# fperezgamonal/flownet2-tf

Hardware: AMD Instinct MI355X
Metric: forward pairs/sec at 512x384 (FlowNet2) (higher is better)
Workload: dtype f16x2 (split fp16 hi+lo operands, 3 fp16 MFMAs per product, fp32 accumulate); 1 GPU; FlowNet2 forward, batch=4 synthetic 512x384 pairs per GPU, seeded synthetic weights; pairs_per_gpu=4, parallelism=dp1 (no collective)

## Files before the change

flownet2-tf_amd/csrc/conv.hip:

```cpp
#include "conv_common.h"
#include <cstdlib>

namespace fn2 {

template <typename T, typename OutT, int TC, int WC, int WP>
__global__ void __launch_bounds__(256) conv_igemm_kernel(const ConvArgs p) {
  constexpr int CH = 16 / (int)sizeof(T);
  constexpr int BC = WC * TC * 16;
  constexpr int BP = WP * 64;
  constexpr int NT = 256;
  static_assert(WC * WP == 4, "4 waves per block");
  constexpr int NPR = BP / 64;
  constexpr int NWR = (BC * 4 + NT - 1) / NT;
  constexpr int WSWZ_BIT = (TC == 4) ? 5 : (TC == 2) ? 4 : 3;
  __shared__ uint4 lds[2][(BC + BP) * 4];

  const int tid = threadIdx.x, lane = tid & 63, wave = tid >> 6;
  const int wc = wave / WP, wp = wave % WP;
  const int cid = tid & 3;

  int pad_y = p.pad, pad_x = p.pad, oy_off = 0, ox_off = 0, osc = 1;
  const T* wgt = reinterpret_cast<const T*>(p.wgt);
  const int phase = blockIdx.z / p.splitk, split = blockIdx.z - phase * p.splitk;
  if (p.deconv) {
// ... 160 lines not shown
  for (int pt = 0; pt < 4; ++pt) {
    const int m = m0 + wp * 64 + pt * 16 + fi;
    if (m >= p.M) continue;
    const int n = m / (p.OH * p.OW);
    const int rem = m - n * (p.OH * p.OW);
    const int oy = rem / p.OW, ox = rem - oy * p.OW;
    OutT* po = out + (((size_t)n * p.out_H + (oy * osc + oy_off)) * p.out_W + (ox * osc + ox_off)) * p.out_cs +
               p.out_c0;
#pragma unroll
    for (int t = 0; t < TC; ++t) {
      float v[4];
      const int co = cout_base + t * 4;
#pragma unroll
      for (int r = 0; r < 4; ++r) {
        float x = acc[t][pt][r] * p.out_scale + bias[t][r];
        if constexpr (sizeof(OutT) == 4) {
          if (p.accum && co + r < p.Cout) x += load_elem<OutT>(po + co + r);
          if (co + r < p.Cout) x = act_grad<OutT>(p, out, po + co + r, co + r, x);
        }
        if (p.act == FN2_ACT_LEAKY) x = leaky(x);
        v[r] = x;
      }
      if (p.vec_ok && co + 3 < p.Cout) {
        store4<OutT>(po + co, v[0], v[1], v[2], v[3]);
      } else {
#pragma unroll
        for (int r = 0; r < 4; ++r)
          if (co + r < p.Cout) store_elem<OutT>(po + co + r, v[r]);
      }
    }
  }
}

template <typename OutT>
__global__ void __launch_bounds__(256) splitk_finalize_kernel(const float* __restrict__ ws, const float* __restrict__ bias,
                                                              OutT* __restrict__ out, long npix, int ws_cs, int splitk,
                                                              int Cout, int out_cs, int out_c0, int act, int vec_ok,
                                                              float out_scale, int accum, const OutT* __restrict__ mask_y,
                                                              int mask_c0, int mask_c1, const float* __restrict__ up_src,
                                                              const float* __restrict__ up_w, const float* __restrict__ up_bias,
                                                              int up_c0, int out_H, int out_W) {
  const int groups = ws_cs / 4;
  const int groups_all = groups + (up_src != nullptr ? 1 : 0);
  const long total = npix * groups_all;
  const size_t slab = (size_t)npix * ws_cs;
  for (long i = (long)blockIdx.x * blockDim.x + threadIdx.x; i < total; i += (long)gridDim.x * blockDim.x) {
    const long pix = i / groups_all;
    const int co = (int)(i - pix * groups_all) * 4;
    if (co == groups * 4) {
      const int ox = (int)(pix % out_W), oy = (int)((pix / out_W) % out_H), n = (int)(pix / out_W / out_H);
      const int H = out_H >> 1, W = out_W >> 1;
      const int a = oy & 1, b = ox & 1, y = oy >> 1, x = ox >> 1;
      float r0 = up_bias ? up_bias[0] : 0.f, r1 = up_bias ? up_bias[1] : 0.f;
#pragma unroll
      for (int ty = 0; ty < 2; ++ty) {
        const int iy = y - 1 + a + ty, ky = 3 - a - 2 * ty;
        if (iy < 0 || iy >= H) continue;
#pragma unroll
        for (int tx = 0; tx < 2; ++tx) {
          const int ix = x - 1 + b + tx, kx = 3 - b - 2 * tx;
          if (ix < 0 || ix >= W) continue;
          const float2 v = *reinterpret_cast<const float2*>(up_src + (((long)n * H + iy) * W + ix) * 2);
          const float* ww = up_w + (ky * 4 + kx) * 4;
          r0 += v.x * ww[0] + v.y * ww[1];
          r1 += v.x * ww[2] + v.y * ww[3];
        }
      }
      OutT* pu = out + (size_t)pix * out_cs + up_c0;
      store_elem<OutT>(pu, r0);
      store_elem<OutT>(pu + 1, r1);
      continue;
    }
    float4 v = *reinterpret_cast<const float4*>(ws + pix * ws_cs + co);
    int s = 1;
    for (; s + 3 < splitk; s += 4) {
      float4 t[4];
#pragma unroll
      for (int u = 0; u < 4; ++u) t[u] = *reinterpret_cast<const float4*>(ws + (s + u) * slab + pix * ws_cs + co);
#pragma unroll
      for (int u = 0; u < 4; ++u) { v.x += t[u].x; v.y += t[u].y; v.z += t[u].z; v.w += t[u].w; }
    }
    for (; s < splitk; ++s) {
      const float4 t = *reinterpret_cast<const float4*>(ws + s * slab + pix * ws_cs + co);
      v.x += t.x; v.y += t.y; v.z += t.z; v.w += t.w;
    }
    float r[4] = {v.x, v.y, v.z, v.w};
    OutT* po = out + (size_t)pix * out_cs + out_c0 + co;
    const bool full = vec_ok && co + 3 < Cout;
    float old[4] = {0.f, 0.f, 0.f, 0.f}, yv[4] = {1.f, 1.f, 1.f, 1.f};
    const bool mask = mask_y != nullptr && co < mask_c1 && co + 4 > mask_c0;
    if constexpr (sizeof(OutT) == 4) {
      if (full) {
        if (accum) load4<OutT>(po, old);
        if (mask) load4<OutT>(mask_y + (size_t)pix * out_cs + out_c0 + co, yv);
      } else {
#pragma unroll
        for (int j = 0; j < 4; ++j)
          if (co + j < Cout) {
            if (accum) old[j] = load_elem<OutT>(po + j);
            if (mask) yv[j] = load_elem<OutT>(mask_y + (size_t)pix * out_cs + out_c0 + co + j);
          }
      }
    }
#pragma unroll
    for (int j = 0; j < 4; ++j) {
      r[j] *= out_scale;
      if (bias != nullptr && co + j < Cout) r[j] += bias[co + j];
      if constexpr (sizeof(OutT) == 4) {
        if (accum) r[j] += old[j];
        if (mask && co + j >= mask_c0 && co + j < mask_c1) r[j] *= yv[j] > 0.f ? 1.f : (yv[j] < 0.f ? 0.1f : 0.55f);
      }
      if (act == FN2_ACT_LEAKY) r[j] = leaky(r[j]);
    }
    if (vec_ok && co + 3 < Cout) {
      store4<OutT>(po, r[0], r[1], r[2], r[3]);
    } else {
#pragma unroll
// ... 179 lines not shown
    for (int idx = tid; idx < HY * HX * 9; idx += 256) {
      const int p = idx / 9, j = idx - p * 9;
      const int hy = p / HX, hx = p - hy * HX;
      const int gy = y0 + hy, gx = x0 + hx;
      float2 v = make_float2(0.f, 0.f);
      if (gy >= 0 && gy < H && gx >= 0 && gx < W)
        v = *reinterpret_cast<const float2*>(t + (((long)n * H + gy) * W + gx) * t_cs + 2 * j);
      sm[idx] = v;
    }
    __syncthreads();
    const int px = tid & (GT_X - 1);
#pragma unroll
    for (int r = 0; r < GT_Y / 4; ++r) {
      const int py = (tid >> 6) + 4 * r;
      const int oy = ty * GT_Y + py, ox = tx * GT_X + px;
      if (oy < H && ox < W) {
        float a0 = b0, a1 = b1;
#pragma unroll
        for (int ky = 0; ky < 3; ++ky)
#pragma unroll
          for (int kx = 0; kx < 3; ++kx) {
            const float2 v = sm[((py + ky) * HX + px + kx) * 9 + ky * 3 + kx];
            a0 += v.x; a1 += v.y;
          }
        *reinterpret_cast<float2*>(out + (((long)n * H + oy) * W + ox) * 2) = make_float2(a0, a1);
      }
    }
    __syncthreads();
  }
}

struct TailSrc { const float* t; int t_cs; int nslab; long slab; float scale; };

template <int NT, int TY, int TX, bool UP, typename OutT>
__global__ void __launch_bounds__(256) head_tail_kernel(const TailSrc ts, const float* __restrict__ bias,
                                                        float* __restrict__ pf, int N, int H, int W, int ring,
                                                        const float* __restrict__ up_w, const float* __restrict__ up_bias,
                                                        OutT* __restrict__ up, int up_cs, int up_c0) {
  constexpr int R = NT / 2, E = UP ? 1 : 0, HALO = R + E;
  constexpr int RW = TX + 2 * HALO, RH = TY + 2 * HALO, NTAP = NT * NT;
  constexpr int EW = TX + 2 * E, EH = TY + 2 * E;
  __shared__ float2 sm[RH * RW * NTAP];
  __shared__ float2 spf[EH * EW];
  __shared__ float sw[64];
  const int tid = threadIdx.x;
  if (UP && tid < 64) sw[tid] = up_w[tid];
  const int tiles_x = (W + TX - 1) / TX, tiles_y = (H + TY - 1) / TY;
  const float b0 = bias ? bias[0] : 0.f, b1 = bias ? bias[1] : 0.f;
  for (int blk = blockIdx.x; blk < N * tiles_y * tiles_x; blk += gridDim.x) {
    const int tx = blk % tiles_x, ty = (blk / tiles_x) % tiles_y, n = blk / (tiles_x * tiles_y);
    const int x0 = tx * TX - HALO, y0 = ty * TY - HALO;
    for (int idx = tid; idx < RH * RW * NTAP; idx += 256) {
      const int p = idx / NTAP, j = idx - p * NTAP;
      const int hy = p / RW, hx = p - hy * RW;
      const int gy = y0 + hy, gx = x0 + hx;
      float2 v = make_float2(0.f, 0.f);
      if (gy >= 0 && gy < H && gx >= 0 && gx < W) {
        const float* src = ts.t + (((long)n * H + gy) * W + gx) * ts.t_cs + 2 * j;
        v = *reinterpret_cast<const float2*>(src);
        for (int sl = 1; sl < ts.nslab; ++sl) {
          const float2 u = *reinterpret_cast<const float2*>(src + sl * ts.slab);
          v.x += u.x; v.y += u.y;
        }
        v.x *= ts.scale; v.y *= ts.scale;
      }
      sm[idx] = v;
    }
    __syncthreads();
    for (int e = tid; e < EH * EW; e += 256) {
      const int ey = e / EW, ex = e - ey * EW;
      const int oy = ty * TY - E + ey, ox = tx * TX - E + ex;
      float a0 = 0.f, a1 = 0.f;
      if (oy >= 0 && oy < H && ox >= 0 && ox < W) {
        const bool inner = ey >= E && ey < E + TY && ex >= E && ex < E + TX;
        float2* po = reinterpret_cast<float2*>(pf + (((long)n * H + oy) * W + ox) * 2);
        if (ring && (oy == 0 || oy == H - 1 || ox == 0 || ox == W - 1)) {
          const float2 v = *po;
          a0 = v.x; a1 = v.y;
        } else {
          a0 = b0; a1 = b1;
#pragma unroll
          for (int ky = 0; ky < NT; ++ky)
#pragma unroll
            for (int kx = 0; kx < NT; ++kx) {
// ... 19 lines not shown
          const int iy = y - 1 + a + tty, ky = 3 - a - 2 * tty;
          const int gy = ty * TY + iy;
          if (gy < 0 || gy >= H) continue;
#pragma unroll
          for (int ttx = 0; ttx < 2; ++ttx) {
            const int ix = x - 1 + b + ttx, kx = 3 - b - 2 * ttx;
            const int gx = tx * TX + ix;
            if (gx < 0 || gx >= W) continue;
            const float2 v = spf[(iy + E) * EW + ix + E];
            const float* ww = sw + (ky * 4 + kx) * 4;
            r0 += v.x * ww[0] + v.y * ww[1];
            r1 += v.x * ww[2] + v.y * ww[3];
          }
        }
        OutT* po = up + (((size_t)n * 2 * H + oy) * 2 * W + ox) * up_cs + up_c0;
        if constexpr (is_x2<OutT>::value) {
          const size_t addr = reinterpret_cast<size_t>(po);
          _Float16* g = reinterpret_cast<_Float16*>(addr & ~size_t(31));
          const int j = (int)((addr & 31) >> 2);
          typedef __attribute__((ext_vector_type(2))) _Float16 h2;
          const _Float16 h0 = (_Float16)r0, h1 = (_Float16)r1;
          *reinterpret_cast<h2*>(g + j) = h2{h0, h1};
          *reinterpret_cast<h2*>(g + 8 + j) = h2{(_Float16)(r0 - (float)h0), (_Float16)(r1 - (float)h1)};
        } else {
          store_elem<OutT>(po, r0);
          store_elem<OutT>(po + 1, r1);
        }
      }
    }
    __syncthreads();
  }
}

__global__ void __launch_bounds__(256) head_ring_kernel(const x2_t* __restrict__ in, int in_cs, int in_c0, int cin_groups,
                                                        const float* __restrict__ wc, const float* __restrict__ bc,
                                                        float* __restrict__ pf, int N, int H, int W) {
  const int lane = threadIdx.x & 63;
  const long wave = ((long)blockIdx.x * blockDim.x + threadIdx.x) >> 6;
  const long nwaves = ((long)gridDim.x * blockDim.x) >> 6;
  const int ring = 2 * W + 2 * (H - 2);
  const int nitems = 25 * cin_groups;
  const size_t case_stride = (size_t)nitems * 8 * 2;
  for (long m = wave; m < (long)N * ring; m += nwaves) {
    const int n = (int)(m / ring), r = (int)(m - (long)n * ring);
    int y, x;
    if (r < W) { y = 0; x = r; }
    else if (r < 2 * W) { y = H - 1; x = r - W; }
    else { const int q = r - 2 * W; y = 1 + (q >> 1); x = (q & 1) ? W - 1 : 0; }
    const int cy = y == 0 ? 0 : (y == H - 1 ? 2 : 1), cx = x == 0 ? 0 : (x == W - 1 ? 2 : 1);
    const int cs = 3 * cy + cx;
    const float* w = wc + (size_t)cs * case_stride;
    float a0 = 0.f, a1 = 0.f;
    for (int q = lane; q < nitems; q += 64) {
      const int tap = q / cin_groups, gi = q - tap * cin_groups;
      const int ky = tap / 5, kx = tap - ky * 5;
      const int iy = y + ky - 2, ix = x + kx - 2;
      if (iy < 0 || iy >= H || ix < 0 || ix >= W) continue;
      const uint4* src = reinterpret_cast<const uint4*>(in + (((size_t)n * H + iy) * W + ix) * in_cs + in_c0 + gi * 8);
      float xv[8];
      join8(src[0], src[1], xv);
      const float* u = w + (size_t)q * 16;
#pragma unroll
      for (int j = 0; j < 8; ++j) {
        a0 += xv[j] * u[2 * j];
        a1 += xv[j] * u[2 * j + 1];
      }
    }
#pragma unroll
    for (int off = 32; off > 0; off >>= 1) {
      a0 += __shfl_xor(a0, off, 64);
      a1 += __shfl_xor(a1, off, 64);
    }
    if (lane == 0)
      *reinterpret_cast<float2*>(pf + (((size_t)n * H + y) * W + x) * 2) = make_float2(a0 + bc[2 * cs], a1 + bc[2 * cs + 1]);
  }
}

template <typename OutT>
__global__ void __launch_bounds__(256) upsample_flow_kernel(const float* __restrict__ in,
                                                            const float* __restrict__ w, const float* __restrict__ bias,
                                                            OutT* __restrict__ out,
                                                            int N, int H, int W, int out_cs, int out_c0) {
  __shared__ float sw[64];
  if (threadIdx.x < 64) sw[threadIdx.x] = w[threadIdx.x];
  __syncthreads();
// ... 81 lines not shown
  if (g > 256L * 16) g = 256L * 16;
  if (g < 1) g = 1;
  return (int)g;
}

static int check_view(const fn2_tensor* t, const char* what) {
  FN2_REQUIRE(t && t->data, "%s: null tensor", what);
  FN2_REQUIRE(t->dtype >= FN2_F32 && t->dtype <= FN2_F16X2, "%s: bad dtype", what);
  FN2_REQUIRE(t->n >= 1 && t->h >= 1 && t->w >= 1 && t->c >= 1, "%s: bad dims", what);
  FN2_REQUIRE(t->c0 >= 0 && t->c0 + t->c <= t->cs, "%s: channel slice outside the buffer", what);
  return FN2_OK;
}

template <int NIMG>
static int pack_imgs(const float* i0, const float* i1, const fn2_tensor* out, int n, int n0, int pad, void* stream) {
  FN2_REQUIRE(pad >= 0 && out->h > 2 * pad && out->w > 2 * pad, "pack: bad border");
  FN2_REQUIRE(out->c0 % 8 == 0 && out->cs % 8 == 0 && out->c0 + 8 <= out->cs, "pack: needs an 8-channel aligned slot");
  const int h = out->h - 2 * pad, w = out->w - 2 * pad;
  const long npix = (long)n * h * w;
  const dim3 g(grid_for(npix, 256)), b(256);
  hipStream_t s = (hipStream_t)stream;
  if (out->dtype == FN2_F32)
    hipLaunchKernelGGL((pack_image_kernel<float, NIMG>), g, b, 0, s, i0, i1, (float*)out->data, n, h, w, n0, pad, out->cs, out->c0);
  else if (out->dtype == FN2_F16X2)
    hipLaunchKernelGGL((pack_image_kernel<x2_t, NIMG>), g, b, 0, s, i0, i1, (x2_t*)out->data, n, h, w, n0, pad, out->cs, out->c0);
  else if (out->dtype == FN2_BF16)
    hipLaunchKernelGGL((pack_image_kernel<bf16_t, NIMG>), g, b, 0, s, i0, i1, (bf16_t*)out->data, n, h, w, n0, pad, out->cs, out->c0);
  else
    hipLaunchKernelGGL((pack_image_kernel<f16_t, NIMG>), g, b, 0, s, i0, i1, (f16_t*)out->data, n, h, w, n0, pad, out->cs, out->c0);
  FN2_CHECK_LAUNCH("pack_image");
  return FN2_OK;
}

template <int NT, int TY, int TX, typename OutT>
void launch_head_tail(bool up, const TailSrc ts, const float* bias, float* pf, int n, int h, int w, int ring,
                      const float* up_w, const float* up_bias, void* up_data, int up_cs, int up_c0, hipStream_t s) {
  const long tiles = (long)n * ((h + TY - 1) / TY) * ((w + TX - 1) / TX);
  const dim3 grid((unsigned)std::min<long>(tiles, 1 << 16)), block(256);
  if (up)
    hipLaunchKernelGGL((head_tail_kernel<NT, TY, TX, true, OutT>), grid, block, 0, s, ts, bias, pf, n, h, w, ring, up_w,
                       up_bias, (OutT*)up_data, up_cs, up_c0);
  else
    hipLaunchKernelGGL((head_tail_kernel<NT, TY, TX, false, float>), grid, block, 0, s, ts, bias, pf, n, h, w, ring,
                       (const float*)nullptr, (const float*)nullptr, (float*)nullptr, 0, 0);
}
template <typename OutT>
void launch_head_tail_t(int taps, bool up, const TailSrc ts, const float* bias, float* pf, int n, int h, int w,
                        int ring, const float* up_w, const float* up_bias, void* up_data, int up_cs, int up_c0,
                        hipStream_t s) {
  const long big = (long)n * ((h + 7) / 8) * ((w + 63) / 64);
  if (taps == 3) {
    if (big >= 256) launch_head_tail<3, 8, 64, OutT>(up, ts, bias, pf, n, h, w, ring, up_w, up_bias, up_data, up_cs, up_c0, s);
    else launch_head_tail<3, 4, 32, OutT>(up, ts, bias, pf, n, h, w, ring, up_w, up_bias, up_data, up_cs, up_c0, s);
  } else {
    if (big >= 256) launch_head_tail<5, 8, 32, OutT>(up, ts, bias, pf, n, h, w, ring, up_w, up_bias, up_data, up_cs, up_c0, s);
    else launch_head_tail<5, 4, 32, OutT>(up, ts, bias, pf, n, h, w, ring, up_w, up_bias, up_data, up_cs, up_c0, s);
  }
}

}

using namespace fn2;

extern "C" {

int fn2_conv2d_plan(int in_dtype, int cin_pad, int cout, fn2_conv_plan* plan) {
  FN2_REQUIRE(plan, "conv2d_plan: null plan");
  FN2_REQUIRE(in_dtype >= FN2_F32 && in_dtype <= FN2_F16X2, "conv2d_plan: bad dtype");
  FN2_REQUIRE(cin_pad > 0 && cin_pad % 8 == 0 && cout >= 1, "conv2d_plan: cin_pad must be a positive multiple of 8");
  const int esz = dtype_size(in_dtype);
  if (cout == 2) {
    plan->layout = 0; plan->cout_tile = 16; plan->kstep_elems = 64 / esz;
    plan->wgt_dtype = in_dtype == FN2_F16X2 ? FN2_F32 : in_dtype;
    return FN2_OK;
  }
  if (conv_fast_ok(in_dtype, cin_pad, cout)) {
    plan->layout = 1; plan->cout_tile = cout > 64 ? 128 : cout > 32 ? 64 : 32; plan->kstep_elems = 128 / esz;
    plan->wgt_dtype = in_dtype;
    return FN2_OK;
  }
  if (in_dtype == FN2_F16X2)
    return fail(FN2_ERR_UNSUPPORTED, "split-fp16 inputs need cin_pad %% 32 == 0 (LDS-DMA kernel); got %d", cin_pad);
  plan->layout = 0; plan->cout_tile = cout > 64 ? 128 : cout > 32 ? 64 : cout > 16 ? 32 : 16;
  plan->kstep_elems = 64 / esz; plan->wgt_dtype = in_dtype;
  return FN2_OK;
}

}

// ... 340 lines not shown
      a.fh_w1 = ha.ksteps * 4 * 4;
      a.fh_groups = ha.cin_chunks >> 1;
      a.fh_bias = ha.bias;
      a.fh_out = reinterpret_cast<float*>(ha.out);
      a.fh_out_cs = ha.out_cs; a.fh_out_c0 = ha.out_c0;
      a.fh_scale = ha.out_scale;
    } else {
      rc = fn2_conv2d(h, stream);
      if (rc) return rc;
    }
  }
  if (d->wgt_layout >= 1) {
    a.ksteps = a.ksteps / 2;
    a.kper = cdiv(a.kper, 2);
    a.splitk = cdiv(a.ksteps, a.kper);
    if (a.splitk == 1) a.ws = nullptr;
    rc = launch_conv_fast(a, d->in.dtype, d->out.dtype, tile, phases, s);
  } else if (d->in.dtype == FN2_F32 && d->out.dtype == FN2_F16X2) rc = launch_conv<float, x2_t>(a, tile, phases, s);
  else if (d->in.dtype == FN2_F32) rc = launch_conv<float, float>(a, tile, phases, s);
  else if (d->in.dtype == FN2_BF16 && d->out.dtype == FN2_BF16) rc = launch_conv<bf16_t, bf16_t>(a, tile, phases, s);
  else if (d->in.dtype == FN2_BF16) rc = launch_conv<bf16_t, float>(a, tile, phases, s);
  else if (d->out.dtype == FN2_F16) rc = launch_conv<f16_t, f16_t>(a, tile, phases, s);
  else rc = launch_conv<f16_t, float>(a, tile, phases, s);
  if (rc || conv_name_sink().buf) return rc;
  if (a.splitk == 1) {
    if (d->up_src == nullptr || a.up_src != nullptr) return rc;
    fn2_tensor uv = d->out;
    uv.c = 2; uv.c0 = d->up_c0;
    return fn2_upsample_flow(d->up_src, d->up_w, d->up_bias, &uv, d->out.n, d->out.h / 2, d->out.w / 2, stream);
  }
  if ((a.dbg & 524288) || d->raw_partials) return rc;
  const long npix = (long)a.N * a.out_H * a.out_W;
  const int fgrid = grid_for(npix * (a.ws_cs / 4 + (d->up_src != nullptr ? 1 : 0)), 256);
  if (d->out.dtype == FN2_F32)
    hipLaunchKernelGGL(splitk_finalize_kernel<float>, dim3(fgrid), dim3(256), 0, s, a.ws, a.bias, (float*)a.out, npix,
                       a.ws_cs, a.splitk, a.Cout, a.out_cs, a.out_c0, a.act, a.vec_ok, a.out_scale, a.accum, (const float*)a.mask_y, a.mask_c0, a.mask_c1, d->up_src, d->up_w, d->up_bias, d->up_c0, a.out_H, a.out_W);
  else if (d->out.dtype == FN2_F16X2)
    hipLaunchKernelGGL(splitk_finalize_kernel<x2_t>, dim3(fgrid), dim3(256), 0, s, a.ws, a.bias, (x2_t*)a.out,
                       npix, a.ws_cs, a.splitk, a.Cout, a.out_cs, a.out_c0, a.act, a.vec_ok, a.out_scale, a.accum, (const x2_t*)a.mask_y, a.mask_c0, a.mask_c1, d->up_src, d->up_w, d->up_bias, d->up_c0, a.out_H, a.out_W);
  else if (d->out.dtype == FN2_BF16)
    hipLaunchKernelGGL(splitk_finalize_kernel<bf16_t>, dim3(fgrid), dim3(256), 0, s, a.ws, a.bias, (bf16_t*)a.out,
                       npix, a.ws_cs, a.splitk, a.Cout, a.out_cs, a.out_c0, a.act, a.vec_ok, a.out_scale, a.accum, (const bf16_t*)a.mask_y, a.mask_c0, a.mask_c1, d->up_src, d->up_w, d->up_bias, d->up_c0, a.out_H, a.out_W);
  else
    hipLaunchKernelGGL(splitk_finalize_kernel<f16_t>, dim3(fgrid), dim3(256), 0, s, a.ws, a.bias, (f16_t*)a.out,
                       npix, a.ws_cs, a.splitk, a.Cout, a.out_cs, a.out_c0, a.act, a.vec_ok, a.out_scale, a.accum, (const f16_t*)a.mask_y, a.mask_c0, a.mask_c1, d->up_src, d->up_w, d->up_bias, d->up_c0, a.out_H, a.out_W);
  FN2_CHECK_LAUNCH("splitk_finalize");
  return FN2_OK;
}

int fn2_flow_head_gather(const float* t, int t_cs, const float* bias, float* out, int n, int h, int w, void* stream) {
  FN2_REQUIRE(t && out, "flow_head_gather: null pointer");
  FN2_REQUIRE(t_cs >= 18 && t_cs % 2 == 0 && n >= 1 && h >= 1 && w >= 1, "flow_head_gather: t must hold 18 partials per pixel");
  const long tiles = (long)n * ((h + GT_Y - 1) / GT_Y) * ((w + GT_X - 1) / GT_X);
  if (tiles >= 1024)
    hipLaunchKernelGGL(flow_head_gather_kernel, dim3((unsigned)std::min<long>(tiles, 1 << 16)), dim3(256), 0,
                       (hipStream_t)stream, t, t_cs, bias, out, n, h, w);
  else
    hipLaunchKernelGGL(flow_head_gather_small_kernel, dim3(grid_for((long)n * h * w, 256)), dim3(256), 0,
                       (hipStream_t)stream, t, t_cs, bias, out, n, h, w);
  FN2_CHECK_LAUNCH("flow_head_gather");
  return FN2_OK;
}

int fn2_flow_head_tail(const float* t, int t_cs, int taps, const float* bias, float* pf, int n, int h, int w, int ring,
                       const float* up_w, const float* up_bias, const fn2_tensor* up_out, void* stream) {
  return fn2_flow_head_tail_slabs(t, t_cs, 1, 0, 1.f, taps, bias, pf, n, h, w, ring, up_w, up_bias, up_out, stream);
}

int fn2_flow_head_tail_slabs(const float* t, int t_cs, int nslab, int64_t slab_stride, float scale, int taps, const float* bias,
                             float* pf, int n, int h, int w, int ring, const float* up_w, const float* up_bias,
                             const fn2_tensor* up_out, void* stream) {
  FN2_REQUIRE(t && pf, "flow_head_tail: null pointer");
  FN2_REQUIRE(nslab >= 1 && (nslab == 1 || slab_stride >= (int64_t)n * h * w * t_cs), "flow_head_tail: bad slab geometry");
  const TailSrc ts{t, t_cs, nslab, (long)slab_stride, scale};
  FN2_REQUIRE(taps == 3 || taps == 5, "flow_head_tail: taps must be 3 or 5");
  FN2_REQUIRE(t_cs >= 2 * taps * taps && t_cs % 2 == 0 && n >= 1 && h >= 1 && w >= 1,
              "flow_head_tail: t must hold 2 * taps^2 partials per pixel");
  FN2_REQUIRE(!ring || (h >= 3 && w >= 3), "flow_head_tail: a border ring needs h, w >= 3");
  const bool up = up_w != nullptr;
  hipStream_t s = (hipStream_t)stream;
  if (!up) {
    launch_head_tail_t<float>(taps, false, ts, bias, pf, n, h, w, ring, nullptr, nullptr, nullptr, 0, 0, s);
  } else {
    int rc = check_view(up_out, "flow_head_tail upsample output");
    if (rc) return rc;
    FN2_REQUIRE(up_out->c == 2 && up_out->n == n && up_out->h == 2 * h && up_out->w == 2 * w,
                "flow_head_tail: the upsample view must be [n, 2h, 2w, 2]");
    if (up_out->dtype == FN2_F16X2) FN2_REQUIRE(up_out->c0 % 2 == 0, "flow_head_tail: split-fp16 slice must start at an even channel");
    void* d = up_out->data;
    if (up_out->dtype == FN2_F32) launch_head_tail_t<float>(taps, true, ts, bias, pf, n, h, w, ring, up_w, up_bias, d, up_out->cs, up_out->c0, s);
    else if (up_out->dtype == FN2_F16X2) launch_head_tail_t<x2_t>(taps, true, ts, bias, pf, n, h, w, ring, up_w, up_bias, d, up_out->cs, up_out->c0, s);
    else if (up_out->dtype == FN2_BF16) launch_head_tail_t<bf16_t>(taps, true, ts, bias, pf, n, h, w, ring, up_w, up_bias, d, up_out->cs, up_out->c0, s);
    else launch_head_tail_t<f16_t>(taps, true, ts, bias, pf, n, h, w, ring, up_w, up_bias, d, up_out->cs, up_out->c0, s);
  }
  FN2_CHECK_LAUNCH("flow_head_tail");
  return FN2_OK;
}

int fn2_flow_head5(const fn2_tensor* x, const void* wgt, int cin_pad, int kpad, float out_scale, const float* bias, float* pf,
// ... 28 lines not shown
  { const char* e = getenv("FN2_H5_DBG"); a.dbg = e ? atoi(e) : 0; }
  a.h5_tiles = (int)blocks;
  long total = blocks;
  if (ring && ring_w != nullptr) {
    FN2_REQUIRE(ring_b != nullptr, "flow_head5: ring_w without ring_b");
    a.h5_wc = ring_w; a.h5_bc = ring_b; a.h5_groups = (x->c + 7) / 8;
    FN2_REQUIRE(x->c0 + a.h5_groups * 8 <= x->cs, "flow_head5: the last 8-channel group reaches past the buffer");
    total += cdiv((long)x->n * (2 * x->w + 2 * (x->h - 2)), 16);
  }
  {
    const char* e = getenv("FN2_H5_STRIP");
    if ((a.ksteps == 3 || a.ksteps == 6) && !(e && atoi(e) == 0) && !(a.dbg & 10)) {
      const int nstrip = cdiv(x->w, 60);
      const char* eb = getenv("FN2_H5_BLOCKS");
      const int target = eb ? atoi(eb) : 256;
      const int segs = std::max(1, std::min(x->h, target / std::max(1, x->n * nstrip)));
      const int rows = cdiv(x->h, segs);
      a.h5_tx = nstrip; a.h5_ty = cdiv(x->h, rows); a.h5_rows = rows;
      return launch_head5_strip(a, x->n * a.h5_ty * a.h5_tx, (hipStream_t)stream);
    }
  }
  return launch_head5(a, (int)total, (hipStream_t)stream);
}

int fn2_flow_head_ring(const fn2_tensor* x, const float* wc, const float* bc, float* pf, void* stream) {
  int rc = check_view(x, "flow_head_ring input");
  if (rc) return rc;
  FN2_REQUIRE(wc && bc && pf, "flow_head_ring: null pointer");
  FN2_REQUIRE(x->dtype == FN2_F16X2 && x->cs % 8 == 0 && x->c0 % 8 == 0, "flow_head_ring: split-fp16 input, 8-aligned view");
  FN2_REQUIRE(x->h >= 3 && x->w >= 3, "flow_head_ring: h, w >= 3");
  const int groups = (x->c + 7) / 8;
  FN2_REQUIRE(x->c0 + groups * 8 <= x->cs, "flow_head_ring: the last 8-channel group reaches past the buffer");
  const long ring = (long)x->n * (2 * x->w + 2 * (x->h - 2));
  hipLaunchKernelGGL(head_ring_kernel, dim3(grid_for(ring * 64, 256)), dim3(256), 0, (hipStream_t)stream, (const x2_t*)x->data,
                     x->cs, x->c0, groups, wc, bc, pf, x->n, x->h, x->w);
  FN2_CHECK_LAUNCH("flow_head_ring");
  return FN2_OK;
}

int fn2_upsample_flow(const float* in, const float* w, const float* bias, const fn2_tensor* out, int n, int h, int wd,
                      void* stream) {
  FN2_REQUIRE(in && w, "upsample_flow: null pointer");
  int rc = check_view(out, "upsample_flow output");
  if (rc) return rc;
  FN2_REQUIRE(out->c == 2 && out->n == n && out->h == 2 * h && out->w == 2 * wd,
              "upsample_flow: output view must be [n, 2h, 2w, 2]");
  const long total = (long)n * 4 * h * wd;
  if (out->dtype == FN2_F32)
    hipLaunchKernelGGL(upsample_flow_kernel<float>, dim3(grid_for(total, 256)), dim3(256), 0, (hipStream_t)stream,
                       in, w, bias, (float*)out->data, n, h, wd, out->cs, out->c0);
  else if (out->dtype == FN2_F16X2)
    hipLaunchKernelGGL(upsample_flow_kernel<x2_t>, dim3(grid_for(total, 256)), dim3(256), 0, (hipStream_t)stream,
                       in, w, bias, (x2_t*)out->data, n, h, wd, out->cs, out->c0);
  else if (out->dtype == FN2_BF16)
    hipLaunchKernelGGL(upsample_flow_kernel<bf16_t>, dim3(grid_for(total, 256)), dim3(256), 0, (hipStream_t)stream,
                       in, w, bias, (bf16_t*)out->data, n, h, wd, out->cs, out->c0);
  else
    hipLaunchKernelGGL(upsample_flow_kernel<f16_t>, dim3(grid_for(total, 256)), dim3(256), 0, (hipStream_t)stream,
                       in, w, bias, (f16_t*)out->data, n, h, wd, out->cs, out->c0);
  FN2_CHECK_LAUNCH("upsample_flow");
  return FN2_OK;
}

int fn2_pack_pair(const float* a, const float* b, const fn2_tensor* out, int pad, void* stream) {
  FN2_REQUIRE(a && b, "pack_pair: null pointer");
  int rc = check_view(out, "pack_pair output");
  if (rc) return rc;
  FN2_REQUIRE(out->c == 6, "pack_pair: output view must have 6 channels");
// ... 37 lines not shown
```

flownet2-tf_amd/src/_hip.py:

```python
import ctypes as C
import os

import numpy as np
import torch

_HERE = os.path.dirname(os.path.abspath(__file__))
LIB_PATH = os.path.join(os.path.dirname(_HERE), "lib", "libflownet2_hip.so")

FN2_F32, FN2_BF16, FN2_F16, FN2_F16X2 = 0, 1, 2, 3
ACT_NONE, ACT_LEAKY = 0, 1
OK = 0
ERR_INVALID_ARGUMENT, ERR_UNSUPPORTED, ERR_HIP = -1, -2, -3
MASK_F32, MASK_U8 = 0, 1


class Fn2Tensor(C.Structure):
    _fields_ = [("data", C.c_void_p), ("dtype", C.c_int32), ("n", C.c_int32), ("h", C.c_int32),
                ("w", C.c_int32), ("c", C.c_int32), ("cs", C.c_int32), ("c0", C.c_int32)]


class Fn2ConvPlan(C.Structure):
    _fields_ = [("layout", C.c_int32), ("cout_tile", C.c_int32), ("kstep_elems", C.c_int32),
                ("wgt_dtype", C.c_int32)]

# ... 22 lines not shown
    "fn2_last_error": (C.c_char_p, []),
    "fn2_version": (_i, []),
    "fn2_crc32c": (C.c_uint32, [_p, C.c_int64, C.c_uint32]),
    "fn2_device_info": (_i, [C.c_char_p, _i, _ip]),
    "fn2_correlation_out_shape": (_i, [_i] * 7 + [_ip] * 3),
    "fn2_correlation_f32": (_i, [_p, _p, _p] + [_i] * 9 + [_p]),
    "fn2_correlation_workspace_bytes": (C.c_int64, [_i] * 9),
    "fn2_correlation_f32_ws": (_i, [_p, _p, _p] + [_i] * 9 + [_p, C.c_int64, _p]),
    "fn2_correlation_f32_kernel_name": (_i, [_i] * 10 + [C.c_char_p, _i]),
    "fn2_correlation_grad_f32": (_i, [_p] * 5 + [_i] * 9 + [_p]),
    "fn2_correlation_grad_f32_kernel_name": (_i, [_i] * 9 + [C.c_char_p, _i]),
    "fn2_flow_warp_f32": (_i, [_p, _p, _p, _i, _i, _i, _i, _p]),
    "fn2_flow_warp_grad_f32": (_i, [_p] * 5 + [_i] * 4 + [_p]),
    "fn2_downsample_f32": (_i, [_p, _p] + [_i] * 6 + [_p]),
    "fn2_downsample_scaled_f32": (_i, [_p, _f, _p] + [_i] * 6 + [_p]),
    "fn2_fill_zero": (_i, [_p, C.c_int64, _p]),
    "fn2_add_f32": (_i, [_p, _p, C.c_int64, _p]),
    "fn2_slice_copy_f32": (_i, [_tp, _p, _p]),
    "fn2_resize_bilinear_f32": (_i, [_p, _p] + [_i] * 6 + [_f, _p]),
    "fn2_conv2d_plan": (_i, [_i, _i, _i, C.POINTER(Fn2ConvPlan)]),
    "fn2_conv2d_workspace_bytes": (C.c_int64, [C.POINTER(Fn2ConvDesc)]),
    "fn2_conv2d": (_i, [C.POINTER(Fn2ConvDesc), _p]),
    "fn2_conv2d_kernel_name": (_i, [C.POINTER(Fn2ConvDesc), C.c_char_p, _i]),
    "fn2_conv2d_splits": (_i, [C.POINTER(Fn2ConvDesc)]),
    "fn2_augment_f32": (_i, [_p, _p, _p, _p, _i, _i, _i, _i, _i, _i, _p]),
    "fn2_flow_augmentation_f32": (_i, [_p, _p, _p, _p, _i, _i, _i, _i, _i, _p]),
    "fn2_selflow_workspace_bytes": (C.c_int64, [_i, _i, _i]),
    "fn2_selflow_stats": (_i, [_p, _p, _p, _p, _p, C.c_int64, _i, _i, _i, _p]),
    "fn2_selflow_apply": (_i, [_p] * 15 + [C.c_int64, _i, _i, _i, _p]),
    "fn2_flow_head_gather": (_i, [_p, _i, _p, _p, _i, _i, _i, _p]),
    "fn2_upsample_flow": (_i, [_p, _p, _p, _tp, _i, _i, _i, _p]),
    "fn2_flow_head_tail": (_i, [_p, _i, _i, _p, _p, _i, _i, _i, _i, _p, _p, _tp, _p]),
    "fn2_flow_head_tail_slabs": (_i, [_p, _i, _i, C.c_int64, _f, _i, _p, _p, _i, _i, _i, _i, _p, _p, _tp, _p]),
    "fn2_flow_head_ring": (_i, [_tp, _p, _p, _p, _p]),
    "fn2_flow_head5": (_i, [_tp, _p, _i, _i, _f, _p, _p, _i, _p, _p, _p]),
    "fn2_u8_to_f32_lut": (_i, [_p, _p, _p, C.c_int64, _p]),
    "fn2_pack_pair": (_i, [_p, _p, _tp, _i, _p]),
    "fn2_pack_interp_u8": (_i, [_p, _p, _p, _p, _p, _tp, _i, _p]),
    "fn2_pack_image": (_i, [_p, _i, _tp, _i, _i, _p]),
    "fn2_pack_image_s2d": (_i, [_p, _i, _i, _i, _tp, _i, _i, _p]),
    "fn2_correlation_fused": (_i, [_tp, _tp, _tp, _i, _i, _i, _p]),
    "fn2_correlation_fused_kernel_name": (_i, [_tp, _tp, _tp, _i, _i, C.c_char_p, _i]),
    "fn2_stack_input": (_i, [_p, _p, _p, _tp, _i, _p]),
    "fn2_fusion_input": (_i, [_p, _p, _p, _p, _tp, _i, _p]),
    "fn2_stack_input_pf": (_i, [_p, _p, _p, _i, _i, _f, _p, _tp, _i, _p]),
    "fn2_fusion_input_pf": (_i, [_p, _p, _p, _f, _p, _p, _f, _p, _i, _i, _tp, _i, _p]),
    "fn2_epe_loss_grad": (_i, [_p, _p, _p, _p, _i, _i, _i, _f, _f, _p]),
    "fn2_epe_loss_grad_weighted": (_i, [_p, _p, _p, _p, _p, _i, _i, _i, _f, _f, _p]),
    "fn2_leaky_bwd": (_i, [_tp, _tp, _p, _p]),
    "fn2_bias_grad": (_i, [_tp, _p, _p]),
    "fn2_gather_f32": (_i, [_p, _p, _p, C.c_int64, _p]),
    "fn2_to_f16x2": (_i, [_p, _p, _p, C.c_int64, _f, _p]),
    "fn2_to_f16x2_frag": (_i, [_p, _p, _p, C.c_int64, _f, _i, _p]),
    "fn2_adam_step": (_i, [_p, _p, _p, _p, C.c_int64, _f, _f, _f, _f, _i, _f, _f, _p]),
    "fn2_adam_step_multi": (_i, [_p, _p, _p, _i, _f, _f, _f, _f, _i, _f, _p]),
    "fn2_adam_step_multi_dev": (_i, [_p, _p, _p, _i, _p, _p]),
    "fn2_upsample_flow_bwd": (_i, [_tp, _p, _p, _p, _p, _i, _p]),
    "fn2_head_bwd_filter": (_i, [_tp, _p, _p, _i, _i, _p]),
    "fn2_head_g18": (_i, [_p, _tp, _p]),
    "fn2_head_bwd_data": (_i, [_p, _p, _tp, _i, _i, _p]),
    "fn2_conv2d_bwd_filter": (_i, [C.POINTER(Fn2BwdwDesc), _p]),
    "fn2_variational_workspace_bytes": (C.c_int64, [_i, _i, _i]),
    "fn2_variational_refine": (_i, [_p, _p, C.c_int64, C.c_int64, _p, C.c_int64, C.c_int64, _i, _i, _i, _f, _f, _f, _f,
                                    _i, _i, _i, _f, _p, C.c_int64, _p]),
    "fn2_tf_warp_f32": (_i, [_p, C.c_int64, C.c_int64, _p, C.c_int64, C.c_int64, _p, _i, _i, _i, _i, _p]),
    "fn2_fb_occlusion": (_i, [_p, _p, C.c_int64, C.c_int64, _p, _p, _i, _i, _i, _i, _f, _f, _p]),
# ... 94 lines not shown
```

include/flownet2_hip.h:

```cpp
#ifndef FLOWNET2_HIP_H_
#define FLOWNET2_HIP_H_

#include <stddef.h>
#include <stdint.h>

#ifdef __cplusplus
extern "C" {
#endif

typedef enum {
  FN2_OK = 0,
  FN2_ERR_INVALID_ARGUMENT = -1,
  FN2_ERR_UNSUPPORTED = -2,
  FN2_ERR_HIP = -3
} fn2_status;

typedef enum { FN2_F32 = 0, FN2_BF16 = 1, FN2_F16 = 2, FN2_F16X2 = 3 } fn2_dtype;

typedef enum { FN2_ACT_NONE = 0, FN2_ACT_LEAKY = 1  } fn2_act;

typedef struct {
  void* data;
  int32_t dtype;
  int32_t n, h, w;
// ... 56 lines not shown
  int32_t cin_pad;
  int32_t cout_pad;
  int32_t kpad;
  int32_t wgt_layout;
  int32_t accumulate;
  float out_scale;
  void* workspace;
  int64_t workspace_bytes;
  const void* act_grad_y;
  int32_t act_grad_c0, act_grad_c1;
  const float* up_src;
  const float* up_w;
  const float* up_bias;
  int32_t up_c0;
  const void* head;
  int32_t raw_partials;
} fn2_conv_desc;

typedef struct {
  int32_t layout, cout_tile, kstep_elems, wgt_dtype;
} fn2_conv_plan;
int fn2_conv2d_plan(int in_dtype, int cin_pad, int cout, fn2_conv_plan* plan);
int64_t fn2_conv2d_workspace_bytes(const fn2_conv_desc* d);
int fn2_conv2d(const fn2_conv_desc* d, void* stream);
int fn2_conv2d_kernel_name(const fn2_conv_desc* desc, char* name, int cap);
int fn2_conv2d_splits(const fn2_conv_desc* desc);

int fn2_flow_head_gather(const float* t, int t_cs, const float* bias, float* out, int n, int h, int w, void* stream);
int fn2_flow_head_tail(const float* t, int t_cs, int taps, const float* bias, float* pf, int n, int h, int w, int ring,
                       const float* up_w, const float* up_bias, const fn2_tensor* up_out, void* stream);
int fn2_flow_head_tail_slabs(const float* t, int t_cs, int nslab, int64_t slab_stride, float scale, int taps, const float* bias,
                             float* pf, int n, int h, int w, int ring, const float* up_w, const float* up_bias,
                             const fn2_tensor* up_out, void* stream);
int fn2_flow_head5(const fn2_tensor* x, const void* wgt, int cin_pad, int kpad, float out_scale, const float* bias, float* pf,
                   int ring, const float* ring_w, const float* ring_b, void* stream);
int fn2_flow_head_ring(const fn2_tensor* x, const float* wc, const float* bc, float* pf, void* stream);
int fn2_upsample_flow(const float* in, const float* w, const float* bias, const fn2_tensor* out, int n, int h, int wd,
                      void* stream);

int fn2_u8_to_f32_lut(const unsigned char* src, const float* lut256, float* dst, long count, void* stream);

int fn2_pack_pair(const float* a, const float* b, const fn2_tensor* out, int pad, void* stream);
int fn2_pack_interp_u8(const unsigned char* img, const unsigned char* mask, const float* sparse, const float* lut256,
                       const unsigned char* flags, const fn2_tensor* out, int pad, void* stream);
int fn2_pack_image(const float* img, int n_img, const fn2_tensor* out, int n0, int pad, void* stream);
int fn2_pack_image_s2d(const float* img, int n_img, int h, int w, const fn2_tensor* out, int n0, int pad, void* stream);

int fn2_correlation_fused(const fn2_tensor* a, const fn2_tensor* b, const fn2_tensor* out,
                          int max_displacement, int stride_2, int act, void* stream);
int fn2_correlation_fused_kernel_name(const fn2_tensor* a, const fn2_tensor* b, const fn2_tensor* out,
                                      int max_displacement, int stride_2, char* name, int cap);

int fn2_stack_input(const float* a, const float* b, const float* flow, const fn2_tensor* out, int pad,
                    void* stream);

int fn2_fusion_input(const float* a, const float* b, const float* flow_sd, const float* flow_css,
                     const fn2_tensor* out, int pad, void* stream);
int fn2_stack_input_pf(const float* a, const float* b, const float* pf, int pf_h, int pf_w, float scale, float* flow_out,
                       const fn2_tensor* out, int pad, void* stream);
int fn2_fusion_input_pf(const float* a, const float* b, const float* pf_sd, float scale_sd, float* flow_sd_out,
                        const float* pf_css, float scale_css, float* flow_css_out, int pf_h, int pf_w,
                        const fn2_tensor* out, int pad, void* stream);


int fn2_epe_loss_grad(const float* pred, const float* label, float* dpred, float* loss_accum, int n, int h, int w,
                      float weight, float grad_mult, void* stream);
// ... 76 lines not shown
```

Before: 1159 pairs/s.

## Batch split-K slab loads in flight for head tail and finalize reductions

Adds a templated slab reduction helper that issues every slab load for several items before any add, so more memory requests are outstanding per thread. By default the head tail kernel uses it, and the small-grid tiles shrink (4x16 or 2x16 instead of 4x32) to launch more blocks. The finalize and ring kernels get in-flight variants that run only when an environment variable is set. This raises register pressure and shifts the order of floating-point sums.

Result: no change. 1158 pairs/s (median of 3 runs) (-0.0%).

```diff
diff --git a/flownet2-tf_amd/csrc/conv.hip b/flownet2-tf_amd/csrc/conv.hip
--- a/flownet2-tf_amd/csrc/conv.hip
+++ b/flownet2-tf_amd/csrc/conv.hip
@@ -216,7 +216,40 @@
   }
 }
 
-template <typename OutT>
+typedef float slab_f2 __attribute__((ext_vector_type(2)));
+typedef float slab_f4 __attribute__((ext_vector_type(4)));
+
+template <int C, int NI, typename V>
+__device__ __forceinline__ void slab_chunk(V (&acc)[NI], const float* const (&src)[NI], size_t slab, int s0, int cnt) {
+  V t[C][NI];
+#pragma unroll
+  for (int u = 0; u < C; ++u)
+#pragma unroll
+    for (int i = 0; i < NI; ++i)
+      t[u][i] = *reinterpret_cast<const V*>(src[i] + (size_t)(s0 + (u < cnt ? u : cnt - 1)) * slab);
+  __builtin_amdgcn_sched_barrier(0);
+#pragma unroll
+  for (int u = 0; u < C; ++u)
+#pragma unroll
+    for (int i = 0; i < NI; ++i) {
+      const V sum = acc[i] + t[u][i];
+      const V next = s0 + u == 0 ? t[u][i] : sum;
+      acc[i] = u < cnt ? next : acc[i];
+    }
+}
+
+template <int CMAX, int NI, typename V>
+__device__ __forceinline__ void slab_sum(V (&acc)[NI], const float* const (&src)[NI], size_t slab, int nslab) {
+  if (nslab == 1) slab_chunk<1, NI, V>(acc, src, slab, 0, 1);
+  else if (nslab == 2) slab_chunk<2, NI, V>(acc, src, slab, 0, 2);
+  else if (nslab <= 4) slab_chunk<4, NI, V>(acc, src, slab, 0, nslab);
+  else if (nslab <= 8) slab_chunk<8, NI, V>(acc, src, slab, 0, nslab);
+  else if (CMAX >= 16 && nslab <= 16) slab_chunk<(CMAX >= 16 ? 16 : 8), NI, V>(acc, src, slab, 0, nslab);
+  else
+    for (int s0 = 0; s0 < nslab; s0 += CMAX) slab_chunk<CMAX, NI, V>(acc, src, slab, s0, nslab - s0 < CMAX ? nslab - s0 : CMAX);
+}
+
+template <typename OutT, bool INFLIGHT>
 __global__ void __launch_bounds__(256) splitk_finalize_kernel(const float* __restrict__ ws, const float* __restrict__ bias,
                                                               OutT* __restrict__ out, long npix, int ws_cs, int splitk,
                                                               int Cout, int out_cs, int out_c0, int act, int vec_ok,
@@ -255,18 +288,26 @@
       store_elem<OutT>(pu + 1, r1);
       continue;
     }
-    float4 v = *reinterpret_cast<const float4*>(ws + pix * ws_cs + co);
-    int s = 1;
-    for (; s + 3 < splitk; s += 4) {
-      float4 t[4];
-#pragma unroll
-      for (int u = 0; u < 4; ++u) t[u] = *reinterpret_cast<const float4*>(ws + (s + u) * slab + pix * ws_cs + co);
-#pragma unroll
-      for (int u = 0; u < 4; ++u) { v.x += t[u].x; v.y += t[u].y; v.z += t[u].z; v.w += t[u].w; }
-    }
-    for (; s < splitk; ++s) {
-      const float4 t = *reinterpret_cast<const float4*>(ws + s * slab + pix * ws_cs + co);
-      v.x += t.x; v.y += t.y; v.z += t.z; v.w += t.w;
+    float4 v;
+    if constexpr (INFLIGHT) {
+      slab_f4 acc[1] = {slab_f4{0.f, 0.f, 0.f, 0.f}};
+      const float* const src[1] = {ws + pix * ws_cs + co};
+      slab_sum<16, 1, slab_f4>(acc, src, slab, splitk);
+      v = make_float4(acc[0].x, acc[0].y, acc[0].z, acc[0].w);
+    } else {
+      v = *reinterpret_cast<const float4*>(ws + pix * ws_cs + co);
+      int s = 1;
+      for (; s + 3 < splitk; s += 4) {
+        float4 t[4];
+#pragma unroll
+        for (int u = 0; u < 4; ++u) t[u] = *reinterpret_cast<const float4*>(ws + (s + u) * slab + pix * ws_cs + co);
+#pragma unroll
+        for (int u = 0; u < 4; ++u) { v.x += t[u].x; v.y += t[u].y; v.z += t[u].z; v.w += t[u].w; }
+      }
+      for (; s < splitk; ++s) {
+        const float4 t = *reinterpret_cast<const float4*>(ws + s * slab + pix * ws_cs + co);
+        v.x += t.x; v.y += t.y; v.z += t.z; v.w += t.w;
+      }
     }
     float r[4] = {v.x, v.y, v.z, v.w};
     OutT* po = out + (size_t)pix * out_cs + out_c0 + co;
@@ -512,7 +553,7 @@
 
 struct TailSrc { const float* t; int t_cs; int nslab; long slab; float scale; };
 
-template <int NT, int TY, int TX, bool UP, typename OutT>
+template <int NT, int TY, int TX, bool UP, typename OutT, bool INFLIGHT>
 __global__ void __launch_bounds__(256) head_tail_kernel(const TailSrc ts, const float* __restrict__ bias,
                                                         float* __restrict__ pf, int N, int H, int W, int ring,
                                                         const float* __restrict__ up_w, const float* __restrict__ up_bias,
@@ -530,6 +571,31 @@
   for (int blk = blockIdx.x; blk < N * tiles_y * tiles_x; blk += gridDim.x) {
     const int tx = blk % tiles_x, ty = (blk / tiles_x) % tiles_y, n = blk / (tiles_x * tiles_y);
     const int x0 = tx * TX - HALO, y0 = ty * TY - HALO;
+    if constexpr (INFLIGHT) {
+      constexpr int NI = 4;
+      for (int base = tid; base < RH * RW * NTAP; base += NI * 256) {
+        const float* src[NI];
+        bool ok[NI];
+        slab_f2 acc[NI];
+#pragma unroll
+        for (int i = 0; i < NI; ++i) {
+          const int idx = base + i * 256;
+          const int p = idx / NTAP, j = idx - p * NTAP;
+          const int hy = p / RW, hx = p - hy * RW;
+          const int gy = y0 + hy, gx = x0 + hx;
+          ok[i] = idx < RH * RW * NTAP && gy >= 0 && gy < H && gx >= 0 && gx < W;
+          src[i] = ok[i] ? ts.t + (((long)n * H + gy) * W + gx) * ts.t_cs + 2 * j : ts.t;
+          acc[i] = slab_f2{0.f, 0.f};
+        }
+        slab_sum<8, NI, slab_f2>(acc, src, (size_t)ts.slab, ts.nslab);
+#pragma unroll
+        for (int i = 0; i < NI; ++i) {
+          const int idx = base + i * 256;
+          if (idx < RH * RW * NTAP)
+            sm[idx] = ok[i] ? make_float2(acc[i].x * ts.scale, acc[i].y * ts.scale) : make_float2(0.f, 0.f);
+        }
+      }
+    } else
     for (int idx = tid; idx < RH * RW * NTAP; idx += 256) {
       const int p = idx / NTAP, j = idx - p * NTAP;
       const int hy = p / RW, hx = p - hy * RW;
@@ -615,6 +681,7 @@
   }
 }
 
+template <bool INFLIGHT>
 __global__ void __launch_bounds__(256) head_ring_kernel(const x2_t* __restrict__ in, int in_cs, int in_c0, int cin_groups,
                                                         const float* __restrict__ wc, const float* __restrict__ bc,
                                                         float* __restrict__ pf, int N, int H, int W) {
@@ -634,6 +701,49 @@
     const int cs = 3 * cy + cx;
     const float* w = wc + (size_t)cs * case_stride;
     float a0 = 0.f, a1 = 0.f;
+    if constexpr (INFLIGHT) {
+      constexpr int NI = 4;
+      for (int q0 = lane; q0 < nitems; q0 += NI * 64) {
+        uint4 xa[NI], xb[NI];
+        float4 u[NI][4];
+        bool ok[NI];
+#pragma unroll
+        for (int i = 0; i < NI; ++i) {
+          const int qi = q0 + i * 64;
+          const int q = qi < nitems ? qi : q0;
+          const int tap = q / cin_groups, gi = q - tap * cin_groups;
+          const int ky = tap / 5, kx = tap - ky * 5;
+          int iy = y + ky - 2, ix = x + kx - 2;
+          const bool in_img = iy >= 0 && iy < H && ix >= 0 && ix < W;
+          ok[i] = qi < nitems && in_img;
+          if (!in_img) { iy = y; ix = x; }
+          const uint4* src = reinterpret_cast<const uint4*>(in + (((size_t)n * H + iy) * W + ix) * in_cs + in_c0 + gi * 8);
+          xa[i] = src[0]; xb[i] = src[1];
+          const float4* uw = reinterpret_cast<const float4*>(w + (size_t)q * 16);
+#pragma unroll
+          for (int k = 0; k < 4; ++k) u[i][k] = uw[k];
+        }
+#pragma unroll
+        for (int i = 0; i < NI; ++i)
+          asm volatile("" : "+v"(xa[i].x), "+v"(xa[i].y), "+v"(xa[i].z), "+v"(xa[i].w), "+v"(xb[i].x), "+v"(xb[i].y),
+                            "+v"(xb[i].z), "+v"(xb[i].w) : : "memory");
+#pragma unroll
+        for (int i = 0; i < NI; ++i) {
+          float xv[8];
+          join8(xa[i], xb[i], xv);
+          const float uu[16] = {u[i][0].x, u[i][0].y, u[i][0].z, u[i][0].w, u[i][1].x, u[i][1].y, u[i][1].z, u[i][1].w,
+                                u[i][2].x, u[i][2].y, u[i][2].z, u[i][2].w, u[i][3].x, u[i][3].y, u[i][3].z, u[i][3].w};
+          float b0 = a0, b1 = a1;
+#pragma unroll
+          for (int j = 0; j < 8; ++j) {
+            b0 += xv[j] * uu[2 * j];
+            b1 += xv[j] * uu[2 * j + 1];
+          }
+          a0 = ok[i] ? b0 : a0;
+          a1 = ok[i] ? b1 : a1;
+        }
+      }
+    } else
     for (int q = lane; q < nitems; q += 64) {
       const int tap = q / cin_groups, gi = q - tap * cin_groups;
       const int ky = tap / 5, kx = tap - ky * 5;
@@ -781,29 +891,67 @@
   return FN2_OK;
 }
 
-template <int NT, int TY, int TX, typename OutT>
+static bool reduce_serial() {
+  const char* e = getenv("FN2_REDUCE_SERIAL");
+  return e && atoi(e) != 0;
+}
+static bool reduce_inflight_all() {
+  const char* e = getenv("FN2_REDUCE_INFLIGHT");
+  return e && atoi(e) != 0 && !reduce_serial();
+}
+
+template <int NT, int TY, int TX, typename OutT, bool INFLIGHT>
 void launch_head_tail(bool up, const TailSrc ts, const float* bias, float* pf, int n, int h, int w, int ring,
                       const float* up_w, const float* up_bias, void* up_data, int up_cs, int up_c0, hipStream_t s) {
   const long tiles = (long)n * ((h + TY - 1) / TY) * ((w + TX - 1) / TX);
   const dim3 grid((unsigned)std::min<long>(tiles, 1 << 16)), block(256);
   if (up)
-    hipLaunchKernelGGL((head_tail_kernel<NT, TY, TX, true, OutT>), grid, block, 0, s, ts, bias, pf, n, h, w, ring, up_w,
-                       up_bias, (OutT*)up_data, up_cs, up_c0);
+    hipLaunchKernelGGL((head_tail_kernel<NT, TY, TX, true, OutT, INFLIGHT>), grid, block, 0, s, ts, bias, pf, n, h, w, ring,
+                       up_w, up_bias, (OutT*)up_data, up_cs, up_c0);
   else
-    hipLaunchKernelGGL((head_tail_kernel<NT, TY, TX, false, float>), grid, block, 0, s, ts, bias, pf, n, h, w, ring,
+    hipLaunchKernelGGL((head_tail_kernel<NT, TY, TX, false, float, INFLIGHT>), grid, block, 0, s, ts, bias, pf, n, h, w, ring,
                        (const float*)nullptr, (const float*)nullptr, (float*)nullptr, 0, 0);
 }
+
+static int head_tail_tile(int taps, int n, int h, int w, int nslab) {
+  const long big = (long)n * ((h + 7) / 8) * ((w + 63) / 64);
+  if (big >= 256) return taps == 3 ? 864 : 832;
+  if (reduce_serial()) return 432;
+  const char* e = getenv("FN2_TAIL_TILE");
+  if (e) {
+    const int t = atoi(e);
+    if (t == 416 || t == 216) return t;
+  }
+  (void)nslab;
+  const long t432 = (long)n * ((h + 3) / 4) * ((w + 31) / 32);
+  return t432 < 256 ? 216 : 416;
+}
+
+template <int NT, typename OutT>
+void launch_head_tail_small(int tile, bool serial, bool up, const TailSrc ts, const float* bias, float* pf, int n, int h,
+                            int w, int ring, const float* up_w, const float* up_bias, void* up_data, int up_cs,
+                            int up_c0, hipStream_t s) {
+  if (serial) launch_head_tail<NT, 4, 32, OutT, false>(up, ts, bias, pf, n, h, w, ring, up_w, up_bias, up_data, up_cs, up_c0, s);
+  else if (tile == 216) launch_head_tail<NT, 2, 16, OutT, true>(up, ts, bias, pf, n, h, w, ring, up_w, up_bias, up_data, up_cs, up_c0, s);
+  else launch_head_tail<NT, 4, 16, OutT, true>(up, ts, bias, pf, n, h, w, ring, up_w, up_bias, up_data, up_cs, up_c0, s);
+}
+
 template <typename OutT>
 void launch_head_tail_t(int taps, bool up, const TailSrc ts, const float* bias, float* pf, int n, int h, int w,
                         int ring, const float* up_w, const float* up_bias, void* up_data, int up_cs, int up_c0,
                         hipStream_t s) {
-  const long big = (long)n * ((h + 7) / 8) * ((w + 63) / 64);
+  const bool serial = reduce_serial();
+  const int tile = head_tail_tile(taps, n, h, w, ts.nslab);
   if (taps == 3) {
-    if (big >= 256) launch_head_tail<3, 8, 64, OutT>(up, ts, bias, pf, n, h, w, ring, up_w, up_bias, up_data, up_cs, up_c0, s);
-    else launch_head_tail<3, 4, 32, OutT>(up, ts, bias, pf, n, h, w, ring, up_w, up_bias, up_data, up_cs, up_c0, s);
+    if (tile == 864) {
+      if (serial) launch_head_tail<3, 8, 64, OutT, false>(up, ts, bias, pf, n, h, w, ring, up_w, up_bias, up_data, up_cs, up_c0, s);
+      else launch_head_tail<3, 8, 64, OutT, true>(up, ts, bias, pf, n, h, w, ring, up_w, up_bias, up_data, up_cs, up_c0, s);
+    } else launch_head_tail_small<3, OutT>(tile, serial, up, ts, bias, pf, n, h, w, ring, up_w, up_bias, up_data, up_cs, up_c0, s);
   } else {
-    if (big >= 256) launch_head_tail<5, 8, 32, OutT>(up, ts, bias, pf, n, h, w, ring, up_w, up_bias, up_data, up_cs, up_c0, s);
-    else launch_head_tail<5, 4, 32, OutT>(up, ts, bias, pf, n, h, w, ring, up_w, up_bias, up_data, up_cs, up_c0, s);
+    if (tile == 832) {
+      if (serial) launch_head_tail<5, 8, 32, OutT, false>(up, ts, bias, pf, n, h, w, ring, up_w, up_bias, up_data, up_cs, up_c0, s);
+      else launch_head_tail<5, 8, 32, OutT, true>(up, ts, bias, pf, n, h, w, ring, up_w, up_bias, up_data, up_cs, up_c0, s);
+    } else launch_head_tail_small<5, OutT>(tile, serial, up, ts, bias, pf, n, h, w, ring, up_w, up_bias, up_data, up_cs, up_c0, s);
   }
 }
 
@@ -1210,18 +1358,25 @@
   if ((a.dbg & 524288) || d->raw_partials) return rc;
   const long npix = (long)a.N * a.out_H * a.out_W;
   const int fgrid = grid_for(npix * (a.ws_cs / 4 + (d->up_src != nullptr ? 1 : 0)), 256);
-  if (d->out.dtype == FN2_F32)
-    hipLaunchKernelGGL(splitk_finalize_kernel<float>, dim3(fgrid), dim3(256), 0, s, a.ws, a.bias, (float*)a.out, npix,
-                       a.ws_cs, a.splitk, a.Cout, a.out_cs, a.out_c0, a.act, a.vec_ok, a.out_scale, a.accum, (const float*)a.mask_y, a.mask_c0, a.mask_c1, d->up_src, d->up_w, d->up_bias, d->up_c0, a.out_H, a.out_W);
-  else if (d->out.dtype == FN2_F16X2)
-    hipLaunchKernelGGL(splitk_finalize_kernel<x2_t>, dim3(fgrid), dim3(256), 0, s, a.ws, a.bias, (x2_t*)a.out,
-                       npix, a.ws_cs, a.splitk, a.Cout, a.out_cs, a.out_c0, a.act, a.vec_ok, a.out_scale, a.accum, (const x2_t*)a.mask_y, a.mask_c0, a.mask_c1, d->up_src, d->up_w, d->up_bias, d->up_c0, a.out_H, a.out_W);
-  else if (d->out.dtype == FN2_BF16)
-    hipLaunchKernelGGL(splitk_finalize_kernel<bf16_t>, dim3(fgrid), dim3(256), 0, s, a.ws, a.bias, (bf16_t*)a.out,
-                       npix, a.ws_cs, a.splitk, a.Cout, a.out_cs, a.out_c0, a.act, a.vec_ok, a.out_scale, a.accum, (const bf16_t*)a.mask_y, a.mask_c0, a.mask_c1, d->up_src, d->up_w, d->up_bias, d->up_c0, a.out_H, a.out_W);
-  else
-    hipLaunchKernelGGL(splitk_finalize_kernel<f16_t>, dim3(fgrid), dim3(256), 0, s, a.ws, a.bias, (f16_t*)a.out,
-                       npix, a.ws_cs, a.splitk, a.Cout, a.out_cs, a.out_c0, a.act, a.vec_ok, a.out_scale, a.accum, (const f16_t*)a.mask_y, a.mask_c0, a.mask_c1, d->up_src, d->up_w, d->up_bias, d->up_c0, a.out_H, a.out_W);
+  const bool serial = !reduce_inflight_all();
+#define FN2_FINALIZE(OutT)                                                                                             \
+  do {                                                                                                                  \
+    if (serial)                                                                                                         \
+      hipLaunchKernelGGL((splitk_finalize_kernel<OutT, false>), dim3(fgrid), dim3(256), 0, s, a.ws, a.bias, (OutT*)a.out, npix, \
+                         a.ws_cs, a.splitk, a.Cout, a.out_cs, a.out_c0, a.act, a.vec_ok, a.out_scale, a.accum,         \
+                         (const OutT*)a.mask_y, a.mask_c0, a.mask_c1, d->up_src, d->up_w, d->up_bias, d->up_c0, a.out_H, \
+                         a.out_W);                                                                                      \
+    else                                                                                                                \
+      hipLaunchKernelGGL((splitk_finalize_kernel<OutT, true>), dim3(fgrid), dim3(256), 0, s, a.ws, a.bias, (OutT*)a.out, npix, \
+                         a.ws_cs, a.splitk, a.Cout, a.out_cs, a.out_c0, a.act, a.vec_ok, a.out_scale, a.accum,         \
+                         (const OutT*)a.mask_y, a.mask_c0, a.mask_c1, d->up_src, d->up_w, d->up_bias, d->up_c0, a.out_H, \
+                         a.out_W);                                                                                      \
+  } while (0)
+  if (d->out.dtype == FN2_F32) FN2_FINALIZE(float);
+  else if (d->out.dtype == FN2_F16X2) FN2_FINALIZE(x2_t);
+  else if (d->out.dtype == FN2_BF16) FN2_FINALIZE(bf16_t);
+  else FN2_FINALIZE(f16_t);
+#undef FN2_FINALIZE
   FN2_CHECK_LAUNCH("splitk_finalize");
   return FN2_OK;
 }
@@ -1243,6 +1398,11 @@
 int fn2_flow_head_tail(const float* t, int t_cs, int taps, const float* bias, float* pf, int n, int h, int w, int ring,
                        const float* up_w, const float* up_bias, const fn2_tensor* up_out, void* stream) {
   return fn2_flow_head_tail_slabs(t, t_cs, 1, 0, 1.f, taps, bias, pf, n, h, w, ring, up_w, up_bias, up_out, stream);
+}
+
+int fn2_flow_head_tail_tile(int taps, int n, int h, int w, int nslab) {
+  if ((taps != 3 && taps != 5) || n < 1 || h < 1 || w < 1 || nslab < 1) return 0;
+  return head_tail_tile(taps, n, h, w, nslab);
 }
 
 int fn2_flow_head_tail_slabs(const float* t, int t_cs, int nslab, int64_t slab_stride, float scale, int taps, const float* bias,
@@ -1337,8 +1497,12 @@
   const int groups = (x->c + 7) / 8;
   FN2_REQUIRE(x->c0 + groups * 8 <= x->cs, "flow_head_ring: the last 8-channel group reaches past the buffer");
   const long ring = (long)x->n * (2 * x->w + 2 * (x->h - 2));
-  hipLaunchKernelGGL(head_ring_kernel, dim3(grid_for(ring * 64, 256)), dim3(256), 0, (hipStream_t)stream, (const x2_t*)x->data,
-                     x->cs, x->c0, groups, wc, bc, pf, x->n, x->h, x->w);
+  if (!reduce_inflight_all())
+    hipLaunchKernelGGL(head_ring_kernel<false>, dim3(grid_for(ring * 64, 256)), dim3(256), 0, (hipStream_t)stream,
+                       (const x2_t*)x->data, x->cs, x->c0, groups, wc, bc, pf, x->n, x->h, x->w);
+  else
+    hipLaunchKernelGGL(head_ring_kernel<true>, dim3(grid_for(ring * 64, 256)), dim3(256), 0, (hipStream_t)stream,
+                       (const x2_t*)x->data, x->cs, x->c0, groups, wc, bc, pf, x->n, x->h, x->w);
   FN2_CHECK_LAUNCH("flow_head_ring");
   return FN2_OK;
 }
diff --git a/flownet2-tf_amd/src/_hip.py b/flownet2-tf_amd/src/_hip.py
--- a/flownet2-tf_amd/src/_hip.py
+++ b/flownet2-tf_amd/src/_hip.py
@@ -78,6 +78,7 @@
     "fn2_upsample_flow": (_i, [_p, _p, _p, _tp, _i, _i, _i, _p]),
     "fn2_flow_head_tail": (_i, [_p, _i, _i, _p, _p, _i, _i, _i, _i, _p, _p, _tp, _p]),
     "fn2_flow_head_tail_slabs": (_i, [_p, _i, _i, C.c_int64, _f, _i, _p, _p, _i, _i, _i, _i, _p, _p, _tp, _p]),
+    "fn2_flow_head_tail_tile": (_i, [_i, _i, _i, _i, _i]),
     "fn2_flow_head_ring": (_i, [_tp, _p, _p, _p, _p]),
     "fn2_flow_head5": (_i, [_tp, _p, _i, _i, _f, _p, _p, _i, _p, _p, _p]),
     "fn2_u8_to_f32_lut": (_i, [_p, _p, _p, C.c_int64, _p]),
diff --git a/include/flownet2_hip.h b/include/flownet2_hip.h
--- a/include/flownet2_hip.h
+++ b/include/flownet2_hip.h
@@ -112,6 +112,7 @@
 int fn2_flow_head_tail_slabs(const float* t, int t_cs, int nslab, int64_t slab_stride, float scale, int taps, const float* bias,
                              float* pf, int n, int h, int w, int ring, const float* up_w, const float* up_bias,
                              const fn2_tensor* up_out, void* stream);
+int fn2_flow_head_tail_tile(int taps, int n, int h, int w, int nslab);
 int fn2_flow_head5(const fn2_tensor* x, const void* wgt, int cin_pad, int kpad, float out_scale, const float* bias, float* pf,
                    int ring, const float* ring_w, const float* ring_b, void* stream);
 int fn2_flow_head_ring(const fn2_tensor* x, const float* wc, const float* bc, float* pf, void* stream);
```
